# Kyubyong/dc_tts

Hardware: NVIDIA H100
Metric: mel_frames_per_sec (higher is better)
Workload: dtype f32 (decode: fp32 FMA; TextEnc/SSRN: fp16x2 split operands on wgmma, fp32 accumulate)

## Files before the change

### dc_tts_b200/csrc/kernels_decode.cu

```cuda
#include "kernels_decode.cuh"
#include "numerics.cuh"
#include "tc_ptx.cuh"

#include <cuda_fp16.h>
#include <atomic>
#include <cstddef>
#include <math.h>

namespace dctts {
using namespace ptx;

namespace {

constexpr int NC = DEC_NC, GMAX = DEC_GMAX, NT = DEC_THREADS, NWARP = NT / 32;
constexpr int XLD = 768;
constexpr int PLD = GMAX * 32 + 16;
constexpr int TC_RA = DEC_PL_PAD;
constexpr int TC_APLANE = 2 * TC_RA * 16;
constexpr int TC_ASTAGE = 2 * TC_APLANE;
constexpr int TC_NSTG = 6;
constexpr int gcd_c(int a, int b) { return b == 0 ? a : gcd_c(b, a % b); }
constexpr unsigned TC_QCYC = NC / gcd_c(NC, TC_NSTG) * TC_NSTG;
constexpr int TC_PR = 24;
constexpr int TC_PTAP = 2 * 2 * TC_PR * 16;
static_assert(3 * TC_PTAP <= TC_ASTAGE, "packed tap images inside a stage");
static_assert(GMAX * NT >= 1024, "red: LayerNorm parameters of the pre-pass");
static_assert(TC_RA == DEC_PL_PAD, "pl_c1 rows are staged as whole slabs");

struct Smem {
    float ring[DEC_NSLOT][NWARP][DEC_REG_F];
    float red[GMAX][NT];
    float xin[2][GMAX][XLD];
    union {
        float pre[2][NC][PLD];
        unsigned char tca[TC_NSTG][TC_ASTAGE];
    };
    float outv[2][GMAX * 32];
    float prm[2][DEC_PRM_F];
    unsigned long long fullw[DEC_NSLOT][NWARP];
    unsigned long long gbar[2];
    unsigned long long sbar[TC_NSTG], abar[TC_NSTG];
    float stat[GMAX][2][2];
    uint32_t tc_baddr[96];
    int n_moved_frames, n_moved_utt;
    DecParams P;
    int p_cur[GMAX], p_prev[GMAX], p_next[GMAX], moved[GMAX];
    int fmoved[2];
    long long prof[DEC_NPROF], prof_last;
    int stop[GMAX], ulen[GMAX], f_end;
};

static_assert(sizeof(Smem) + 128 <= 232448, "decode kernel: shared memory budget (227 KB per CTA)");
static_assert(offsetof(Smem, tca) + sizeof(Smem::tca) + 128 * 16 <= sizeof(Smem), "A tile reads past the stages");

#define LAP(i) do { if constexpr (PROF) { if (threadIdx.x == 0) { const long long now_ = clock64(); S.prof[i] += now_ - S.prof_last; S.prof_last = now_; } } } while (0)
enum { LP_START = 0, LP_WAIT = 1, LP_GEMV = 2, LP_RELEASE = 3, LP_GATHER = 4, LP_CBAR = 5, LP_LN = 6, LP_MIX = 7, LP_ATT = 8,
       LP_PYR_ATT = 9, LP_PYR_WTS = 10, LP_PYR_TABLE = 11, LP_PYR_STAGE = 12, LP_PYR_DRAIN = 13, LP_PYR_REFILL = 14,
       LP_PYR_LN = 15, LP_PYR_BAR = 16, LP_FRAME = 17,
       LP_WG_AWAIT = 18, LP_WG_MMA = 19, LP_WG_EPI = 20, LP_COUNT };
static_assert(LP_COUNT <= DEC_NPROF, "lap buckets");

__device__ __forceinline__ float sigmoid_fast(float x) { return __fdividef(1.0f, 1.0f + __expf(-x)); }

__device__ __forceinline__ void cp_async16(void* dst, const void* src, bool valid) {
    const int sz = valid ? 16 : 0;
    asm volatile("cp.async.cg.shared.global [%0], [%1], 16, %2;" :: "r"(smem_u32(dst)), "l"(src), "r"(sz) : "memory");
}
__device__ __forceinline__ void cp_async_commit() { asm volatile("cp.async.commit_group;" ::: "memory"); }
template <int N> __device__ __forceinline__ void cp_async_wait() { asm volatile("cp.async.wait_group %0;" :: "n"(N) : "memory"); }

__device__ __forceinline__ void bulk_g2s(void* dst, const void* src, uint32_t bytes, unsigned long long* bar) {
    asm volatile("cp.async.bulk.shared::cluster.global.mbarrier::complete_tx::bytes [%0], [%1], %2, [%3];"
                 :: "r"(smem_u32(dst)), "l"(src), "r"(bytes), "r"(smem_u32(bar)) : "memory");
}
__device__ __forceinline__ void bulk_g2s_mc(void* dst, const void* src, uint32_t bytes, unsigned long long* bar, uint16_t mask) {
    asm volatile("cp.async.bulk.shared::cluster.global.mbarrier::complete_tx::bytes.multicast::cluster [%0], [%1], %2, [%3], %4;"
                 :: "r"(smem_u32(dst)), "l"(src), "r"(bytes), "r"(smem_u32(bar)), "h"(mask) : "memory");
}
__device__ __forceinline__ void bulk_s2peer(uint32_t dst_cluster, const void* src, uint32_t bytes, uint32_t bar_cluster) {
    asm volatile("cp.async.bulk.shared::cluster.shared::cta.mbarrier::complete_tx::bytes [%0], [%1], %2, [%3];"
                 :: "r"(dst_cluster), "r"(smem_u32(src)), "r"(bytes), "r"(bar_cluster) : "memory");
}
__device__ __forceinline__ void cluster_sync_all() { cluster_arrive(); cluster_wait(); }
__device__ __forceinline__ void fence_proxy_async_global() { asm volatile("fence.proxy.async.global;" ::: "memory"); }

__device__ __forceinline__ size_t pl_idx(int nslab, int rows, int b, int c, int t) {
    return ((size_t)(b * nslab + (c >> 4)) * 4 + ((c >> 3) & 1)) * (size_t)rows * 8 + (size_t)(t + DEC_PL_PAD) * 8 + (c & 7);
}
__device__ __forceinline__ float2 ffma2(float2 a, float2 b, float2 c) { return make_float2(fmaf(a.x, b.x, c.x), fmaf(a.y, b.y, c.y)); }
__device__ __forceinline__ float4 ldcg4(const float* p) { return __ldcg(reinterpret_cast<const float4*>(p)); }
__device__ __forceinline__ uint64_t* bar64(unsigned long long* p) { return reinterpret_cast<uint64_t*>(p); }

struct Cur { int f, seg, c; };
__device__ __forceinline__ void cur_next(const DecParams& P, const Smem& S, Cur& u) {
    u.c++;
    const int end = (u.seg == 0) ? P.nch_enc : (u.seg == 1 ? P.pyr_ch1 : P.nch);
    if (u.c < end) return;
    if (u.seg == 0) {
        if (S.fmoved[u.f & 1]) { u.seg = 1; u.c = P.pyr_ch0; } else { u.seg = 2; u.c = P.nch_enc; }
    } else if (u.seg == 1) { u.seg = 2; u.c = P.nch_enc; }
    else { u.f++; u.seg = 0; u.c = 0; }
}
struct Stream {
    const float* base;
    Cur prod;
    unsigned pos;
    unsigned tcq;
};
template <bool STOP>
__device__ __forceinline__ void stream_issue(const DecParams& P, Smem& S, const Stream& st, const Cur& u, int slot, int warp) {
    if (u.f >= (STOP ? S.f_end : P.steps)) return;
    const DecChunk& ch = P.C[u.c];
    const uint32_t bytes = (uint32_t)ch.nfl4 * 2u;
    mbar_expect_tx(bar64(&S.fullw[slot][warp]), bytes);
    const int off = (u.seg == 1) ? ch.off16 : ch.off;
    bulk_g2s(&S.ring[slot][warp][0], st.base + off + warp * (ch.nfl4 >> 1), bytes, &S.fullw[slot][warp]);
}
__device__ __forceinline__ void stream_advance(const DecParams& P, const Smem& S, Stream& st) {
    cur_next(P, S, st.prod); st.pos++;
}
template <bool STOP>
__device__ __forceinline__ void warp_release(const DecParams& P, Smem& S, Stream& st, int warp, int lane) {
    __syncwarp();
    if (lane == 0) stream_issue<STOP>(P, S, st, st.prod, (int)(st.pos % DEC_NSLOT), warp);
    stream_advance(P, S, st);
}

__device__ __forceinline__ void prefetch_params(const DecParams& P, Smem& S, int li, int rank) {
    const DecLayer& l = P.L[li];
    float* dst = S.prm[li & 1];
    const int tid = threadIdx.x;
    cp_async16(dst + tid * 4, P.lnp[li] + tid * 4, true);
    if ((l.cs & 3) == 0) {
        if (tid < l.ns / 4) {
            const int n = tid * 4;
            cp_async16(dst + 1024 + n, P.bias[li] + ((l.kind == 1 && n >= l.cs) ? l.cout + rank * l.cs + (n - l.cs) : rank * l.cs + n), true);
        }
    } else if (tid < l.ns) {
        dst[1024 + tid] = (tid < l.cs) ? __ldg(P.bias[li] + rank * l.cs + tid) : 0.f;
    }
}
__device__ __forceinline__ void prefetch_taps(const DecParams& P, Smem& S, int li, int j, int b0, int G, int buf) {
    const DecLayer& l = P.L[li];
    if (l.ntaps != 3 || !P.in_hist[li]) return;
    for (int i = threadIdx.x; i < G * 128; i += NT) {
        const int c4 = i & 63, tap = (i >> 6) & 1, g = i >> 7;
        const int t = j - (2 - tap) * l.rate;
        const float* src = P.in_hist[li] + ((size_t)(b0 + g) * P.T + (t < 0 ? 0 : t)) * 256 + c4 * 4;
        cp_async16(&S.xin[buf][g][tap * 256 + c4 * 4], src, t >= 0);
    }
}

template <int GT>
__device__ __forceinline__ void gemv_warp(const float* __restrict__ wreg, const float* __restrict__ x, int kr8, int ns, float (&acc)[GT]) {
    const int lane = threadIdx.x & 31;
    const int lg = (ns == 32) ? 5 : (ns == 16 ? 4 : 3);
    const int n = lane & (ns - 1), sg = lane >> lg;
    const int kper = kr8 >> (5 - lg);
    const float* w = wreg + ((size_t)((sg * kper) >> 2) * ns + n) * 4;
    const float* xs = x + sg * kper;
    const int wstep = ns * 4;
    float2 p0[GT], p1[GT];
#pragma unroll
    for (int g = 0; g < GT; ++g) { p0[g] = make_float2(acc[g], 0.f); p1[g] = make_float2(0.f, 0.f); }
#pragma unroll 2
    for (int k = 0; k < kper; k += 8) {
        const float4 w0 = *reinterpret_cast<const float4*>(w);
        const float4 w1 = *reinterpret_cast<const float4*>(w + wstep);
        w += 2 * wstep;
#pragma unroll
        for (int g = 0; g < GT; ++g) {
            const float4 x0 = *reinterpret_cast<const float4*>(xs + g * XLD + k);
            const float4 x1 = *reinterpret_cast<const float4*>(xs + g * XLD + k + 4);
            float2 a = p0[g], c = p1[g];
            a = ffma2(make_float2(x0.x, x0.y), make_float2(w0.x, w0.y), a);
            c = ffma2(make_float2(x1.x, x1.y), make_float2(w1.x, w1.y), c);
            a = ffma2(make_float2(x0.z, x0.w), make_float2(w0.z, w0.w), a);
            c = ffma2(make_float2(x1.z, x1.w), make_float2(w1.z, w1.w), c);
            p0[g] = a; p1[g] = c;
        }
    }
#pragma unroll
    for (int g = 0; g < GT; ++g) acc[g] = (p0[g].x + p0[g].y) + (p1[g].x + p1[g].y);
}


template <int GT>
__device__ __forceinline__ void gemv_warp32(const float* __restrict__ wreg, const float* __restrict__ x, int kr8, float2 (&pe)[GT],
                                            float2 (&po)[GT]) {
    const int lane = threadIdx.x & 31, cp = lane & 15, kh = lane >> 4;
    const float* w = wreg + (kh * 16 + cp) * 4;
    const float* xs = x + kh * 4;
#pragma unroll 2
    for (int k = 0; k < kr8; k += 8) {
        const float4 wa = *reinterpret_cast<const float4*>(w);
        const float4 wb = *reinterpret_cast<const float4*>(w + 128);
        w += 256;
#pragma unroll
        for (int g = 0; g < GT; ++g) {
            const float4 xv = *reinterpret_cast<const float4*>(xs + g * XLD + k);
            float2 a = pe[g], c = po[g];
            a = ffma2(make_float2(xv.x, xv.y), make_float2(wa.x, wa.y), a);
            c = ffma2(make_float2(xv.x, xv.y), make_float2(wb.x, wb.y), c);
            a = ffma2(make_float2(xv.z, xv.w), make_float2(wa.z, wa.w), a);
            c = ffma2(make_float2(xv.z, xv.w), make_float2(wb.z, wb.w), c);
            pe[g] = a; po[g] = c;
        }
    }
}


template <bool PROF, int GT, bool STOP>
__device__ __forceinline__ int layer_row(const DecParams& P, Smem& S, Stream& st, int li, int j, int b0, int G, int rank, int cb, unsigned& lcount) {
    const DecLayer& l = P.L[li];
    const int tid = threadIdx.x, warp = tid >> 5, lane = tid & 31;
    const bool last = (li + 1 == P.nl);
    const int nl_next = last ? 0 : li + 1;
    const int pb = (int)(lcount & 1u);
    const uint32_t gpar = (lcount >> 1) & 1u;
    const uint32_t gbytes = (uint32_t)(GT * l.ns * 4);

    cp_async_wait<0>();
    __syncthreads();
    if (tid == 0) mbar_expect_tx(bar64(&S.gbar[pb]), NC * gbytes);
    if (!last || j + 1 < P.steps) {
        prefetch_params(P, S, nl_next, rank);
        if (nl_next != P.n_enc) prefetch_taps(P, S, nl_next, last ? j + 1 : j, b0, G, cb ^ 1);
    }
    cp_async_commit();
    LAP(LP_START);

    if (l.ns == 32) {
        float2 pe[GT], po[GT];
#pragma unroll
        for (int g = 0; g < GT; ++g) { pe[g] = make_float2(0.f, 0.f); po[g] = make_float2(0.f, 0.f); }
        for (int c = 0; c < l.nch; ++c) {
            const DecChunk& ch = P.C[l.ch0 + c];
            const int slot = (int)(st.pos % DEC_NSLOT);
            mbar_wait(bar64(&S.fullw[slot][warp]), (st.pos / DEC_NSLOT) & 1u);
            LAP(LP_WAIT);
            const int kr8 = ch.krows >> 3;
            gemv_warp32<GT>(&S.ring[slot][warp][0], &S.xin[cb][0][ch.k0 + warp * kr8], kr8, pe, po);
            LAP(LP_GEMV);
            warp_release<STOP>(P, S, st, warp, lane);
            LAP(LP_RELEASE);
        }
#pragma unroll
        for (int g = 0; g < GT; ++g) {
            float e = pe[g].x + pe[g].y, o = po[g].x + po[g].y;
            e += __shfl_xor_sync(0xffffffffu, e, 16);
            o += __shfl_xor_sync(0xffffffffu, o, 16);
            if (lane < 16) *reinterpret_cast<float2*>(&S.red[g][warp * 32 + 2 * lane]) = make_float2(e, o);
        }
    } else {
        float acc[GT];
#pragma unroll
        for (int g = 0; g < GT; ++g) acc[g] = 0.f;
        for (int c = 0; c < l.nch; ++c) {
            const DecChunk& ch = P.C[l.ch0 + c];
            const int slot = (int)(st.pos % DEC_NSLOT);
            mbar_wait(bar64(&S.fullw[slot][warp]), (st.pos / DEC_NSLOT) & 1u);
            LAP(LP_WAIT);
            const int kr8 = ch.krows >> 3;
            gemv_warp<GT>(&S.ring[slot][warp][0], &S.xin[cb][0][ch.k0 + warp * kr8], kr8, l.ns, acc);
            LAP(LP_GEMV);
            warp_release<STOP>(P, S, st, warp, lane);
            LAP(LP_RELEASE);
        }
#pragma unroll
        for (int g = 0; g < GT; ++g) S.red[g][tid] = acc[g];
    }
    __syncthreads();
    const int lgns = (l.ns == 32) ? 5 : (l.ns == 16 ? 4 : 3);
    {
        const int nvals = GT << lgns, ng = NT >> lgns;
        float* ov = S.outv[pb];
        if (tid < nvals) {
            const float* bs = S.prm[li & 1] + 1024;
            const int g = tid >> lgns, n = tid & (l.ns - 1);
            const float* rp = &S.red[g][n];
            float s0 = bs[n], s1 = 0.f;
#pragma unroll 4
            for (int q = 0; q < ng; q += 2) { s0 += rp[q << lgns]; s1 += rp[(q + 1) << lgns]; }
            ov[tid] = s0 + s1;
            fence_proxy_async_smem();
        }
        if (GT > 1) __syncthreads(); else __syncwarp();
        if (tid < NC)
            bulk_s2peer(mapa(smem_u32(&S.pre[pb][rank][0]), (uint32_t)tid), ov, gbytes, mapa(smem_u32(&S.gbar[pb]), (uint32_t)tid));
    }
    LAP(LP_GATHER);
    mbar_wait(bar64(&S.gbar[pb]), gpar);
    LAP(LP_CBAR);
    {
        const int C = l.cout, cs = l.cs, nh = l.kind + 1;
        const float rC = (C == 256) ? (1.0f / 256.0f) : __frcp_rn((float)C);
        auto pre_off = [&](int c) { const int rk = (cs == 16) ? (c >> 4) : ((c * 205) >> 10); return rk * PLD + (c - rk * cs); };
        for (int pr = warp; pr < GT * nh; pr += NWARP) {
            const int g = (nh == 2) ? (pr >> 1) : pr, hf = (nh == 2) ? (pr & 1) : 0;
            const float* base = &S.pre[pb][0][(g << lgns) + hf * cs];
            const float piv = base[0];
            float sv = 0.f, qv = 0.f;
#pragma unroll
            for (int i = 0; i < 8; ++i) {
                const int c = lane + 32 * i;
                if (c < C) { const float d = base[pre_off(c)] - piv; sv += d; qv = fmaf(d, d, qv); }
            }
#pragma unroll
            for (int o = 16; o > 0; o >>= 1) { sv += __shfl_xor_sync(0xffffffffu, sv, o); qv += __shfl_xor_sync(0xffffffffu, qv, o); }
            if (lane == 0) {
                const float m = sv * rC;
                S.stat[g][hf][0] = piv + m;
                S.stat[g][hf][1] = rsqrtf(fmaxf(qv * rC - m * m, 0.f) + 1e-12f);
            }
        }
        __syncthreads();
        LAP(LP_LN);
        const float* prm = S.prm[li & 1];
        const int cur_off = (l.ntaps - 1) * 256;
        const int next_off = (last || li + 1 == P.n_enc) ? 0 : (P.L[li + 1].ntaps - 1) * 256;
        float* oh = P.out_hist[li];
        __half* pl = last ? nullptr : P.pl_hist[li + 1];
        const int c = tid;
        if (c < C) {
            const int po = pre_off(c);
            const bool mine = (po / PLD == rank) && oh;
            const size_t pl_lo = (size_t)P.pl_rows * 16;
            const float g1 = prm[c], b1 = prm[256 + c], g2 = prm[512 + c], b2 = prm[768 + c];
            float o[GT];
#pragma unroll
            for (int g = 0; g < GT; ++g) {
                const float* pr = &S.pre[pb][0][g << lgns];
                o[g] = (pr[po] - S.stat[g][0][0]) * S.stat[g][0][1] * g1 + b1;
            }
            if (l.kind == 1) {
#pragma unroll
                for (int g = 0; g < GT; ++g) {
                    const float* pr = &S.pre[pb][0][g << lgns];
                    const float h2 = (pr[po + cs] - S.stat[g][1][0]) * S.stat[g][1][1] * g2 + b2;
                    const float h1 = sigmoid_fast(o[g]);
                    o[g] = h1 * h2 + (1.0f - h1) * S.xin[cb][g][cur_off + c];
                }
            } else if (l.act == 1) {
#pragma unroll
                for (int g = 0; g < GT; ++g) o[g] = fmaxf(o[g], 0.f);
            }
#pragma unroll
            for (int g = 0; g < GT; ++g) {
                const size_t row = (size_t)(b0 + g) * P.T + j;
                if (mine && g < G) {
                    oh[row * C + c] = o[g];
                    if (pl) {
                        const size_t ix = pl_idx(C >> 4, P.pl_rows, b0 + g, c, j);
                        split_f16(o[g], pl[ix], pl[ix + pl_lo]);
                    }
                }
                if (last) {
                    o[g] = sigmoid_fast(o[g]);
                    if (rank == 0 && g < G) P.ybuf[row * C + c] = o[g];
                }
                S.xin[cb ^ 1][g][next_off + c] = (g < G) ? o[g] : 0.f;
            }
        } else if (last && c < 128) {
#pragma unroll
            for (int g = 0; g < GT; ++g) S.xin[cb ^ 1][g][c] = 0.f;
        }
    }
    LAP(LP_MIX);
    lcount++;
    return cb ^ 1;
}

__device__ __forceinline__ int attend_row(const DecParams& P, const float (&qv)[8], int b, int p, int lane, float (&ctx)[8]) {
    const int d = P.d;
    const int n_lo = min(max(p, 0), P.N - 1), n_hi = min(n_lo + P.win_size, P.N);
    const float scale = rsqrtf((float)d);
    float sc[4] = {0.f, 0.f, 0.f, 0.f};
#pragma unroll
    for (int i = 0; i < 4; ++i) {
        const int n = n_lo + i;
        if (n < n_hi) {
            const float* k = P.kv + ((size_t)b * P.N + n) * (2 * d) + lane * 8;
            const float4 k0 = ldcg4(k), k1 = ldcg4(k + 4);
            float s = 0.f;
            s = fmaf(qv[0], k0.x, s); s = fmaf(qv[1], k0.y, s); s = fmaf(qv[2], k0.z, s); s = fmaf(qv[3], k0.w, s);
            s = fmaf(qv[4], k1.x, s); s = fmaf(qv[5], k1.y, s); s = fmaf(qv[6], k1.z, s); s = fmaf(qv[7], k1.w, s);
            sc[i] = warp_sum(s) * scale;
        }
    }
    const int cnt = n_hi - n_lo;
    float mx = -INFINITY;
#pragma unroll
    for (int i = 0; i < 4; ++i) if (i < cnt) mx = fmaxf(mx, sc[i]);
    float sum = 0.f;
#pragma unroll
    for (int i = 0; i < 4; ++i) if (i < cnt) { sc[i] = expf(sc[i] - mx); sum += sc[i]; }
    float best = -1.f; int besti = 0;
#pragma unroll
    for (int i = 0; i < 4; ++i) if (i < cnt) { sc[i] = sc[i] / sum; if (sc[i] > best) { best = sc[i]; besti = i; } }
#pragma unroll
    for (int i = 0; i < 8; ++i) ctx[i] = 0.f;
#pragma unroll
    for (int i = 0; i < 4; ++i) {
        const int n = n_lo + i;
        if (n < n_hi) {
            const float* v = P.kv + ((size_t)b * P.N + n) * (2 * d) + d + lane * 8;
            const float4 v0 = ldcg4(v), v1 = ldcg4(v + 4);
            const float p_ = sc[i];
            ctx[0] = fmaf(p_, v0.x, ctx[0]); ctx[1] = fmaf(p_, v0.y, ctx[1]); ctx[2] = fmaf(p_, v0.z, ctx[2]); ctx[3] = fmaf(p_, v0.w, ctx[3]);
            ctx[4] = fmaf(p_, v1.x, ctx[4]); ctx[5] = fmaf(p_, v1.y, ctx[5]); ctx[6] = fmaf(p_, v1.z, ctx[6]); ctx[7] = fmaf(p_, v1.w, ctx[7]);
        }
    }
    return n_lo + besti;
}

struct PreRows { unsigned mask; int t_lo, n, total; };
__device__ __forceinline__ PreRows pre_rows(const Smem& S, int G, int j, int prow) {
    PreRows r;
    r.mask = 0;
#pragma unroll
    for (int g = 0; g < GMAX; ++g) if (g < G && S.moved[g]) r.mask |= 1u << g;
    r.t_lo = max(0, j - (prow - 1));
// ... 520 lines not shown
```

### dc_tts_b200/csrc/tc_ptx.cuh

```cuda
#pragma once
#include <cuda_runtime.h>
#include <stdint.h>

namespace dctts { namespace ptx {

__device__ __forceinline__ uint32_t smem_u32(const void* p) {
    return static_cast<uint32_t>(__cvta_generic_to_shared(p));
}
__device__ __forceinline__ bool elect_one() {
    uint32_t pred = 0;
    asm volatile("{\n\t.reg .pred P;\n\telect.sync _|P, 0xffffffff;\n\tselp.u32 %0, 1, 0, P;\n\t}" : "=r"(pred));
    return pred != 0;
}

__device__ __forceinline__ void mbar_init(uint64_t* bar, uint32_t count) {
    asm volatile("mbarrier.init.shared::cta.b64 [%0], %1;" :: "r"(smem_u32(bar)), "r"(count));
}
__device__ __forceinline__ void fence_mbar_init() { asm volatile("fence.mbarrier_init.release.cluster;" ::: "memory"); }
__device__ __forceinline__ void mbar_expect_tx(uint64_t* bar, uint32_t bytes) {
    asm volatile("mbarrier.arrive.expect_tx.shared::cta.b64 _, [%0], %1;" :: "r"(smem_u32(bar)), "r"(bytes) : "memory");
}
__device__ __forceinline__ bool mbar_try_wait(uint64_t* bar, uint32_t parity) {
    uint32_t ok;
    asm volatile(
        "{\n\t.reg .pred P;\n\t"
        "mbarrier.try_wait.parity.shared::cta.b64 P, [%1], %2;\n\t"
        "selp.u32 %0, 1, 0, P;\n\t}"
        : "=r"(ok) : "r"(smem_u32(bar)), "r"(parity) : "memory");
    return ok != 0;
}
__device__ __forceinline__ void mbar_wait(uint64_t* bar, uint32_t parity) {
    if (mbar_try_wait(bar, parity)) return;
    const long long t0 = clock64();
    while (!mbar_try_wait(bar, parity))
        if (clock64() - t0 > 4000000000ll) __trap();
}

__device__ __forceinline__ void prefetch_tmap(const void* tmap) {
    asm volatile("prefetch.tensormap [%0];" :: "l"(reinterpret_cast<uint64_t>(tmap)) : "memory");
}
__device__ __forceinline__ void tma_load_2d(const void* tmap, uint64_t* bar, void* dst, int c0, int c1) {
    asm volatile("cp.async.bulk.tensor.2d.shared::cluster.global.mbarrier::complete_tx::bytes [%0], [%1, {%3, %4}], [%2];"
                 :: "r"(smem_u32(dst)), "l"(reinterpret_cast<uint64_t>(tmap)), "r"(smem_u32(bar)), "r"(c0), "r"(c1)
                 : "memory");
}
__device__ __forceinline__ void tma_load_3d(const void* tmap, uint64_t* bar, void* dst, int c0, int c1, int c2) {
    asm volatile("cp.async.bulk.tensor.3d.shared::cluster.global.mbarrier::complete_tx::bytes [%0], [%1, {%3, %4, %5}], [%2];"
                 :: "r"(smem_u32(dst)), "l"(reinterpret_cast<uint64_t>(tmap)), "r"(smem_u32(bar)), "r"(c0), "r"(c1), "r"(c2)
                 : "memory");
}

__device__ __forceinline__ void tma_load_3d_mc(const void* tmap, uint64_t* bar, void* dst, int c0, int c1, int c2, uint16_t mask) {
    asm volatile("cp.async.bulk.tensor.3d.shared::cluster.global.mbarrier::complete_tx::bytes.multicast::cluster [%0], [%1, {%3, %4, %5}], [%2], %6;"
                 :: "r"(smem_u32(dst)), "l"(reinterpret_cast<uint64_t>(tmap)), "r"(smem_u32(bar)), "r"(c0), "r"(c1), "r"(c2), "h"(mask)
                 : "memory");
}

__device__ __forceinline__ void tma_store_3d(const void* tmap, const void* src, int c0, int c1, int c2) {
    asm volatile("cp.async.bulk.tensor.3d.global.shared::cta.bulk_group [%0, {%2, %3, %4}], [%1];"
                 :: "l"(reinterpret_cast<uint64_t>(tmap)), "r"(smem_u32(src)), "r"(c0), "r"(c1), "r"(c2) : "memory");
}
__device__ __forceinline__ void tma_store_commit_and_wait() {
    asm volatile("cp.async.bulk.commit_group;" ::: "memory");
    asm volatile("cp.async.bulk.wait_group.read 0;" ::: "memory");
}
__device__ __forceinline__ void fence_proxy_async_smem() { asm volatile("fence.proxy.async.shared::cta;" ::: "memory"); }

__device__ __forceinline__ void wg_fence() { asm volatile("wgmma.fence.sync.aligned;" ::: "memory"); }
__device__ __forceinline__ void wg_commit() { asm volatile("wgmma.commit_group.sync.aligned;" ::: "memory"); }
template <int N>
__device__ __forceinline__ void wg_wait() { asm volatile("wgmma.wait_group.sync.aligned %0;" :: "n"(N) : "memory"); }
template <int R>
__device__ __forceinline__ void wg_fence_regs(float (&d)[R]) {
#pragma unroll
    for (int i = 0; i < R; ++i) asm volatile("" : "+f"(d[i]) :: "memory");
}

#define DCTTS_WG_D8(o) "+f"(d[o + 0]), "+f"(d[o + 1]), "+f"(d[o + 2]), "+f"(d[o + 3]), "+f"(d[o + 4]), "+f"(d[o + 5]), "+f"(d[o + 6]), "+f"(d[o + 7])
template <int NQ, int R>
__device__ __forceinline__ void wgmma_f16(float (&d)[R], uint64_t da, uint64_t db, uint32_t accumulate) {
    static_assert(NQ >= 1 && NQ <= 4 && 8 * NQ <= R, "wgmma_f16: 16..64 columns");
    if constexpr (NQ == 1) {
        asm volatile("{\n\t.reg .pred p;\n\tsetp.ne.b32 p, %10, 0;\n\t"
                     "wgmma.mma_async.sync.aligned.m64n16k16.f32.f16.f16 {%0,%1,%2,%3,%4,%5,%6,%7}, %8, %9, p, 1, 1, 0, 0;\n\t}"
                     : DCTTS_WG_D8(0) : "l"(da), "l"(db), "r"(accumulate));
    } else if constexpr (NQ == 2) {
        asm volatile("{\n\t.reg .pred p;\n\tsetp.ne.b32 p, %18, 0;\n\t"
                     "wgmma.mma_async.sync.aligned.m64n32k16.f32.f16.f16 {%0,%1,%2,%3,%4,%5,%6,%7,%8,%9,%10,%11,%12,%13,%14,%15},"
                     " %16, %17, p, 1, 1, 0, 0;\n\t}"
                     : DCTTS_WG_D8(0), DCTTS_WG_D8(8) : "l"(da), "l"(db), "r"(accumulate));
    } else if constexpr (NQ == 3) {
        asm volatile("{\n\t.reg .pred p;\n\tsetp.ne.b32 p, %26, 0;\n\t"
                     "wgmma.mma_async.sync.aligned.m64n48k16.f32.f16.f16 {%0,%1,%2,%3,%4,%5,%6,%7,%8,%9,%10,%11,%12,%13,%14,%15,"
                     "%16,%17,%18,%19,%20,%21,%22,%23}, %24, %25, p, 1, 1, 0, 0;\n\t}"
                     : DCTTS_WG_D8(0), DCTTS_WG_D8(8), DCTTS_WG_D8(16) : "l"(da), "l"(db), "r"(accumulate));
    } else {
        asm volatile("{\n\t.reg .pred p;\n\tsetp.ne.b32 p, %34, 0;\n\t"
                     "wgmma.mma_async.sync.aligned.m64n64k16.f32.f16.f16 {%0,%1,%2,%3,%4,%5,%6,%7,%8,%9,%10,%11,%12,%13,%14,%15,"
                     "%16,%17,%18,%19,%20,%21,%22,%23,%24,%25,%26,%27,%28,%29,%30,%31}, %32, %33, p, 1, 1, 0, 0;\n\t}"
                     : DCTTS_WG_D8(0), DCTTS_WG_D8(8), DCTTS_WG_D8(16), DCTTS_WG_D8(24) : "l"(da), "l"(db), "r"(accumulate));
    }
}
template <int N>
__device__ __forceinline__ void wgmma_full(float (&d)[N / 2], uint64_t da, uint64_t db, uint32_t accumulate) {
    static_assert(N == 64 || N == 80 || N == 144 || N == 256, "wgmma_full: unsupported width");
    if constexpr (N == 64) {
        asm volatile("{\n\t.reg .pred p;\n\tsetp.ne.b32 p, %34, 0;\n\t"
                     "wgmma.mma_async.sync.aligned.m64n64k16.f32.f16.f16 {%0,%1,%2,%3,%4,%5,%6,%7,%8,%9,%10,%11,%12,%13,%14,%15,%16,%17,%18,%19,%20,%21,%22,%23,%24,%25,%26,%27,%28,%29,%30,%31},"
                     " %32, %33, p, 1, 1, 0, 0;\n\t}"
                     : DCTTS_WG_D8(0), DCTTS_WG_D8(8), DCTTS_WG_D8(16), DCTTS_WG_D8(24) : "l"(da), "l"(db), "r"(accumulate));
    } else if constexpr (N == 80) {
        asm volatile("{\n\t.reg .pred p;\n\tsetp.ne.b32 p, %42, 0;\n\t"
                     "wgmma.mma_async.sync.aligned.m64n80k16.f32.f16.f16 {%0,%1,%2,%3,%4,%5,%6,%7,%8,%9,%10,%11,%12,%13,%14,%15,%16,%17,%18,%19,%20,%21,%22,%23,%24,%25,%26,%27,%28,%29,%30,%31,%32,%33,%34,%35,%36,%37,%38,%39},"
                     " %40, %41, p, 1, 1, 0, 0;\n\t}"
                     : DCTTS_WG_D8(0), DCTTS_WG_D8(8), DCTTS_WG_D8(16), DCTTS_WG_D8(24), DCTTS_WG_D8(32) : "l"(da), "l"(db), "r"(accumulate));
    } else if constexpr (N == 144) {
        asm volatile("{\n\t.reg .pred p;\n\tsetp.ne.b32 p, %74, 0;\n\t"
                     "wgmma.mma_async.sync.aligned.m64n144k16.f32.f16.f16 {%0,%1,%2,%3,%4,%5,%6,%7,%8,%9,%10,%11,%12,%13,%14,%15,%16,%17,%18,%19,%20,%21,%22,%23,%24,%25,%26,%27,%28,%29,%30,%31,%32,%33,%34,%35,%36,%37,%38,%39,%40,%41,%42,%43,%44,%45,%46,%47,%48,%49,%50,%51,%52,%53,%54,%55,%56,%57,%58,%59,%60,%61,%62,%63,%64,%65,%66,%67,%68,%69,%70,%71},"
// ... 76 lines not shown
```

### dc_tts_b200/engine.py

```python
import ctypes as C
import warnings

import numpy as np
import torch

from . import _lib
from .hyperparams import Hyperparams as hp
from .params import check_params


class DcttsError(RuntimeError):
    pass


def _ptr(t):
    return C.c_void_p(0) if t is None else C.c_void_p(t.data_ptr())


def _require_tensors(who, want):
    for t, shape, dt in want:
        if tuple(t.shape) != shape or t.dtype != dt or not t.is_cuda or not t.is_contiguous():
            raise DcttsError("%s: expected a contiguous CUDA %s tensor of shape %s, got %s %s" %
                             (who, dt, shape, t.dtype, tuple(t.shape)))

# ... 11 lines not shown
        h = _lib.Handle()
        torch.cuda.init()
        with torch.cuda.device(self.device):
            torch.zeros(1, device=self.device)
            rc = self._lib.dctts_create(C.byref(st), device, C.byref(h))
        if rc != 0:
            raise DcttsError("dctts_create: " + self._lib.dctts_last_error(None).decode())
        self._h = h
        self.params_loaded = False

    def close(self):
        if getattr(self, "_h", None):
            self._lib.dctts_destroy(self._h)
            self._h = None

    def __del__(self):
        try:
            self.close()
        except Exception:
            pass

    def _check(self, rc, what):
        if rc != 0:
            raise DcttsError("%s: %s" % (what, self._lib.dctts_last_error(self._h).decode()))

    def _stream(self):
        return C.c_void_p(torch.cuda.current_stream(self.device).cuda_stream)

    def _f32(self, x):
        if isinstance(x, np.ndarray):
            x = torch.from_numpy(np.ascontiguousarray(x, dtype=np.float32))
        return x.to(device=self.device, dtype=torch.float32).contiguous()

    def _i32(self, x):
        if isinstance(x, np.ndarray):
            x = torch.from_numpy(np.ascontiguousarray(x, dtype=np.int32))
        return torch.as_tensor(x).to(device=self.device, dtype=torch.int32).contiguous()

    def _empty(self, *shape, dtype=torch.float32):
        return torch.empty(shape, device=self.device, dtype=dtype)

    def stage_params(self, params):
        for name, arr in params.items():
            a = np.ascontiguousarray(arr, dtype=np.float32)
            shape = (C.c_int64 * a.ndim)(*a.shape)
            self._check(self._lib.dctts_set_param(self._h, name.encode(), a.ctypes.data_as(C.c_void_p),
                                                   shape, a.ndim), "dctts_set_param(%s)" % name)

    def commit_params(self):
        self._check(self._lib.dctts_commit_params(self._h), "dctts_commit_params")
        self.params_loaded = True
        return int(self._lib.dctts_num_params(self._h))

    def load_params(self, params):
        check_params(params)
        self.stage_params(params)
        return self.commit_params()

    def restore(self, text2mel_dir, ssrn_dir=None):
        from .checkpoint import Saver, latest_checkpoint
        Saver(var_list=["Text2Mel"]).restore(self, latest_checkpoint(text2mel_dir))
        Saver(var_list=["SSRN", "gs"]).restore(self, latest_checkpoint(ssrn_dir if ssrn_dir is not None else text2mel_dir))
        return self.commit_params()

    def set_tensor_path(self, mode):
        self._check(self._lib.dctts_set_tensor_path(self._h, int(mode)), "dctts_set_tensor_path")

    def set_option(self, name, value):
        self._check(self._lib.dctts_set_option(self._h, name.encode(), int(value)), "dctts_set_option(%s)" % name)

    def get_option(self, name):
        v = C.c_int32(0)
        self._check(self._lib.dctts_get_option(self._h, name.encode(), C.byref(v)), "dctts_get_option(%s)" % name)
        return int(v.value)

    def decode_stats(self):
        a, b, c = C.c_int32(0), C.c_int32(0), C.c_int32(0)
        self._check(self._lib.dctts_decode_stats(self._h, C.byref(a), C.byref(b), C.byref(c)), "dctts_decode_stats")
        return int(a.value), int(b.value), int(c.value)

    def decode_profile(self):
        names = ["start", "stream_wait", "gemv", "release", "gather", "cluster_barrier", "layernorm", "mix", "attention",
                 "re_attention", "re_weights", "re_table", "re_stage", "re_drain", "re_refill", "re_layernorm", "re_barriers",
                 "frame", "wg_a_wait", "wg_mma", "wg_epilogue"]
        v = (C.c_int64 * len(names))()
        self._check(self._lib.dctts_decode_profile(self._h, v, len(names)), "dctts_decode_profile")
        return dict(zip(names, [int(x) for x in v]))

    def reserve(self, batch):
        self._check(self._lib.dctts_reserve(self._h, int(batch)), "dctts_reserve")

    def bench_block(self, scope, B, L, iters=5, warmup=2):
        ms = (C.c_float * 8)()
        n = C.c_int32(0)
        self._check(self._lib.dctts_bench_block(self._h, scope.encode(), B, L, iters, warmup, ms, C.byref(n),
                                                self._stream()), "dctts_bench_block")
        return [float(ms[i]) for i in range(n.value)]

    def conv_gemm(self, impl, mode, X, K, Wd, N, shifts, out, bias=None, accumulate=0):
        ts = [X, Wd, out] + ([bias] if bias is not None else [])
        if not all(t.is_cuda and t.dtype == torch.float32 and t.stride(-1) == 1 for t in ts):
            raise DcttsError("conv_gemm: CUDA float32 tensors with a unit inner stride expected")
        B, L = X.shape[0], X.shape[1]
        rows_ok = X.stride(0) == L * X.stride(1) and (mode == 1 or out.stride(0) == L * out.stride(1))
        taps_ok = (Wd.stride(0) == K * Wd.stride(1)) if mode == 0 else (out.stride(0) == K * out.stride(1))
        dy_ok = mode == 0 or (Wd.shape[0] == B and Wd.shape[1] == L and Wd.stride(0) == L * Wd.stride(1))
        if not (rows_ok and taps_ok and dy_ok):
            raise DcttsError("conv_gemm: rows or taps of a tensor are not evenly pitched")
        sh = (C.c_int32 * len(shifts))(*[int(s) for s in shifts])
        self._check(self._lib.dctts_conv_gemm(self._h, int(impl), int(mode), _ptr(X), X.stride(1), B, L, int(K), _ptr(Wd),
                                              Wd.stride(1), int(N), len(shifts), sh, _ptr(bias), int(accumulate), _ptr(out),
                                              out.stride(1), self._stream()), "dctts_conv_gemm")
        return out

    @staticmethod
    def _pitched(who, ts, rows):
        if not all(t.is_cuda and t.dtype == torch.float32 and t.stride(-1) == 1 for t in ts):
            raise DcttsError("%s: CUDA float32 tensors with a unit inner stride expected" % who)
        pitches = []
        for t in ts:
            lead = t.shape[:-1]
            n = 1
            for s in lead:
                n *= s
            ld = t.stride(-2) if t.dim() >= 2 else t.shape[-1]
            even = all(t.stride(i) == t.stride(i + 1) * t.shape[i + 1] for i in range(t.dim() - 2))
            if n != rows or not even:
                raise DcttsError("%s: rows of a tensor are not evenly pitched, or not %d of them" % (who, rows))
            pitches.append(ld)
        return pitches

    def block_bwd(self, mode, act, C, pre, gout, ln, dy, dparams, X=None, gin=None, dropout_rate=0.0, layer=0, seed=0):
        nconv = 2 * C if mode == 1 else C
        if mode == 1 and (X is None or gin is None):
            raise DcttsError("block_bwd: a highway block (mode 1) needs X and gin")
        rows = 1
        for s in pre.shape[:-1]:
            rows *= s
        ts = [pre, gout, dy] + ([X, gin] if mode == 1 else [])
        if any(t.shape[-1] < w for t, w in zip(ts, (nconv, C, nconv, C, C))):
            raise DcttsError("block_bwd: pre and dy need %d columns, gout, X and gin %d" % (nconv, C))
        lds = self._pitched("block_bwd", ts, rows)
        if gout.stride(-2) != lds[1] or (mode == 1 and gin.stride(-2) != lds[1]):
            raise DcttsError("block_bwd: gout and gin share one pitch")
        if dy.stride(-2) != lds[0]:
            raise DcttsError("block_bwd: pre and dy share one pitch")
        _require_tensors("block_bwd", [(ln, (4, C), torch.float32), (dparams, (4 * C + nconv,), torch.float32)])
        self._check(self._lib.dctts_block_bwd(self._h, int(mode), int(act), rows, int(C), _ptr(pre), lds[0], _ptr(gout), lds[1],
                                              _ptr(X), lds[3] if mode == 1 else 0, _ptr(ln), float(dropout_rate), int(layer),
                                              int(seed) & 0xffffffff, _ptr(dy), _ptr(gin), _ptr(dparams), self._stream()),
                    "dctts_block_bwd")
        return dy

    def attn_bwd(self, gR, Q, KV, align, gts, n_lim, t_lim, gQ, gKV, sums):
        B, T, N, d = align.shape[0], align.shape[2], align.shape[1], self.hp.d
        f32 = torch.float32
        _require_tensors("attn_bwd", [(gR, (B, T, 2 * d), f32), (Q, (B, T, d), f32), (KV, (B, N, 2 * d), f32),
                                      (align, (B, N, T), f32), (gQ, (B, T, d), f32), (gKV, (B, N, 2 * d), f32),
                                      (sums, (3,), torch.float64)])
        if gts.dim() != 2 or gts.shape[0] < n_lim or gts.shape[1] < t_lim:
            raise DcttsError("attn_bwd: gts must be 2-D with at least n_lim = %d rows and t_lim = %d columns, got %s"
                             % (n_lim, t_lim, tuple(gts.shape)))
        ld_gts = self._pitched("attn_bwd", [gts], gts.shape[0])[0]
        self._check(self._lib.dctts_attn_bwd(self._h, _ptr(gR), _ptr(Q), _ptr(KV), _ptr(align), _ptr(gts), ld_gts, B, T, N,
                                             int(n_lim), int(t_lim), _ptr(gQ), _ptr(gKV), _ptr(sums), self._stream()),
                    "dctts_attn_bwd")
        return gQ, gKV
# ... 492 lines not shown
```

Before: 141,100.

## Scatter decode partials with st.async and merge LayerNorm stats per rank

Replaces the staged outv buffer and bulk shared-to-peer copy with direct per-thread st.async pushes of the reduced values into every cluster rank's pre buffer. Each rank also computes local mean/M2 partials via warp shuffles and sends them, so the LayerNorm statistics are merged with a Chan-style combine instead of a separate warp pass, a __syncthreads and a stat array. Parameter and tap prefetch is moved after the gather so it overlaps the cluster barrier wait, which now uses a cluster-scope acquire. This trades a block barrier and an smem round-trip for many small remote stores and extra shuffle work.

```diff
diff --git a/dc_tts_b200/csrc/kernels_decode.cu b/dc_tts_b200/csrc/kernels_decode.cu
--- a/dc_tts_b200/csrc/kernels_decode.cu
+++ b/dc_tts_b200/csrc/kernels_decode.cu
@@ -15,6 +15,7 @@
 constexpr int NC = DEC_NC, GMAX = DEC_GMAX, NT = DEC_THREADS, NWARP = NT / 32;
 constexpr int XLD = 768;
 constexpr int PLD = GMAX * 32 + 16;
+constexpr int PPD = 2 * NC + 4;
 constexpr int TC_RA = DEC_PL_PAD;
 constexpr int TC_APLANE = 2 * TC_RA * 16;
 constexpr int TC_ASTAGE = 2 * TC_APLANE;
@@ -32,15 +33,16 @@
     float red[GMAX][NT];
     float xin[2][GMAX][XLD];
     union {
-        float pre[2][NC][PLD];
+        struct {
+            float pre[2][NC][PLD];
+            float part[2][GMAX * 2][PPD];
+        };
         unsigned char tca[TC_NSTG][TC_ASTAGE];
     };
-    float outv[2][GMAX * 32];
     float prm[2][DEC_PRM_F];
     unsigned long long fullw[DEC_NSLOT][NWARP];
     unsigned long long gbar[2];
     unsigned long long sbar[TC_NSTG], abar[TC_NSTG];
-    float stat[GMAX][2][2];
     uint32_t tc_baddr[96];
     int n_moved_frames, n_moved_utt;
     DecParams P;
@@ -52,12 +54,15 @@
 
 static_assert(sizeof(Smem) + 128 <= 232448, "decode kernel: shared memory budget (227 KB per CTA)");
 static_assert(offsetof(Smem, tca) + sizeof(Smem::tca) + 128 * 16 <= sizeof(Smem), "A tile reads past the stages");
+static_assert(offsetof(Smem, pre) % 16 == 0 && (PLD * 4) % 16 == 0, "pre: 16-byte st.async targets");
+static_assert(offsetof(Smem, part) % 16 == 0 && (PPD * 4) % 16 == 0, "part: float4 loads of the merge");
 
 #define LAP(i) do { if constexpr (PROF) { if (threadIdx.x == 0) { const long long now_ = clock64(); S.prof[i] += now_ - S.prof_last; S.prof_last = now_; } } } while (0)
 enum { LP_START = 0, LP_WAIT = 1, LP_GEMV = 2, LP_RELEASE = 3, LP_GATHER = 4, LP_CBAR = 5, LP_LN = 6, LP_MIX = 7, LP_ATT = 8,
        LP_PYR_ATT = 9, LP_PYR_WTS = 10, LP_PYR_TABLE = 11, LP_PYR_STAGE = 12, LP_PYR_DRAIN = 13, LP_PYR_REFILL = 14,
        LP_PYR_LN = 15, LP_PYR_BAR = 16, LP_FRAME = 17,
-       LP_WG_AWAIT = 18, LP_WG_MMA = 19, LP_WG_EPI = 20, LP_COUNT };
+       LP_WG_AWAIT = 18, LP_WG_MMA = 19, LP_WG_EPI = 20,
+       LP_PREFETCH = 21, LP_COUNT };
 static_assert(LP_COUNT <= DEC_NPROF, "lap buckets");
 
 __device__ __forceinline__ float sigmoid_fast(float x) { return __fdividef(1.0f, 1.0f + __expf(-x)); }
@@ -76,10 +81,6 @@
 __device__ __forceinline__ void bulk_g2s_mc(void* dst, const void* src, uint32_t bytes, unsigned long long* bar, uint16_t mask) {
     asm volatile("cp.async.bulk.shared::cluster.global.mbarrier::complete_tx::bytes.multicast::cluster [%0], [%1], %2, [%3], %4;"
                  :: "r"(smem_u32(dst)), "l"(src), "r"(bytes), "r"(smem_u32(bar)), "h"(mask) : "memory");
-}
-__device__ __forceinline__ void bulk_s2peer(uint32_t dst_cluster, const void* src, uint32_t bytes, uint32_t bar_cluster) {
-    asm volatile("cp.async.bulk.shared::cluster.shared::cta.mbarrier::complete_tx::bytes [%0], [%1], %2, [%3];"
-                 :: "r"(dst_cluster), "r"(smem_u32(src)), "r"(bytes), "r"(bar_cluster) : "memory");
 }
 __device__ __forceinline__ void cluster_sync_all() { cluster_arrive(); cluster_wait(); }
 __device__ __forceinline__ void fence_proxy_async_global() { asm volatile("fence.proxy.async.global;" ::: "memory"); }
@@ -218,16 +219,12 @@
     const int nl_next = last ? 0 : li + 1;
     const int pb = (int)(lcount & 1u);
     const uint32_t gpar = (lcount >> 1) & 1u;
-    const uint32_t gbytes = (uint32_t)(GT * l.ns * 4);
+    const int nh = l.kind + 1;
+    const uint32_t gbytes = (uint32_t)(GT * l.ns * 4), pbytes = (uint32_t)(GT * nh * 8);
 
     cp_async_wait<0>();
     __syncthreads();
-    if (tid == 0) mbar_expect_tx(bar64(&S.gbar[pb]), NC * gbytes);
-    if (!last || j + 1 < P.steps) {
-        prefetch_params(P, S, nl_next, rank);
-        if (nl_next != P.n_enc) prefetch_taps(P, S, nl_next, last ? j + 1 : j, b0, G, cb ^ 1);
-    }
-    cp_async_commit();
+    if (tid == 0) mbar_expect_tx(bar64(&S.gbar[pb]), NC * (gbytes + pbytes));
     LAP(LP_START);
 
     if (l.ns == 32) {
@@ -272,50 +269,88 @@
     }
     __syncthreads();
     const int lgns = (l.ns == 32) ? 5 : (l.ns == 16 ? 4 : 3);
+    const int cs = l.cs;
     {
         const int nvals = GT << lgns, ng = NT >> lgns;
-        float* ov = S.outv[pb];
-        if (tid < nvals) {
-            const float* bs = S.prm[li & 1] + 1024;
+        if ((tid & ~31) < nvals) {
             const int g = tid >> lgns, n = tid & (l.ns - 1);
-            const float* rp = &S.red[g][n];
-            float s0 = bs[n], s1 = 0.f;
+            float v = 0.f;
+            if (tid < nvals) {
+                const float* bs = S.prm[li & 1] + 1024;
+                const float* rp = &S.red[g][n];
+                float s0 = bs[n], s1 = 0.f;
 #pragma unroll 4
-            for (int q = 0; q < ng; q += 2) { s0 += rp[q << lgns]; s1 += rp[(q + 1) << lgns]; }
-            ov[tid] = s0 + s1;
-            fence_proxy_async_smem();
-        }
-        if (GT > 1) __syncthreads(); else __syncwarp();
-        if (tid < NC)
-            bulk_s2peer(mapa(smem_u32(&S.pre[pb][rank][0]), (uint32_t)tid), ov, gbytes, mapa(smem_u32(&S.gbar[pb]), (uint32_t)tid));
+                for (int q = 0; q < ng; q += 2) { s0 += rp[q << lgns]; s1 += rp[(q + 1) << lgns]; }
+                v = s0 + s1;
+            }
+            const int W = (l.ns == 8) ? 8 : 16, w = lane & (W - 1);
+            const float piv = __shfl_sync(0xffffffffu, v, lane & ~(W - 1));
+            const float d = (w < cs) ? v - piv : 0.f;
+            float s1 = d, s2 = d * d;
+#pragma unroll
+            for (int o = 1; o < 8; o <<= 1) { s1 += __shfl_xor_sync(0xffffffffu, s1, o); s2 += __shfl_xor_sync(0xffffffffu, s2, o); }
+            if (W == 16) { s1 += __shfl_xor_sync(0xffffffffu, s1, 8); s2 += __shfl_xor_sync(0xffffffffu, s2, 8); }
+            const float md = s1 * ((cs == 16) ? (1.0f / 16.0f) : __frcp_rn((float)cs));
+            const float mr = piv + md, m2 = fmaxf(fmaf(-s1, md, s2), 0.f);
+            const int q0 = lane & ~3;
+            const float4 v4 = make_float4(__shfl_sync(0xffffffffu, v, q0), __shfl_sync(0xffffffffu, v, q0 + 1),
+                                          __shfl_sync(0xffffffffu, v, q0 + 2), __shfl_sync(0xffffffffu, v, q0 + 3));
+            if (tid < nvals) {
+                const uint32_t bar = smem_u32(&S.gbar[pb]);
+                const uint32_t vdst = smem_u32(&S.pre[pb][rank][(g << lgns) + (n & ~3)]);
+                const int hf = (l.ns == 32) ? (n >> 4) : 0;
+                const uint32_t pdst = smem_u32(&S.part[pb][2 * g + hf][2 * rank]);
+#pragma unroll
+                for (int i = 0; i < NC / 4; ++i) {
+                    const uint32_t r = (uint32_t)((lane & 3) + 4 * i);
+                    st_async_v4(mapa(vdst, r), v4, mapa(bar, r));
+                }
+                for (int r = w; r < NC; r += W) st_async_v2(mapa(pdst, (uint32_t)r), mr, m2, mapa(bar, (uint32_t)r));
+            }
+        }
     }
     LAP(LP_GATHER);
-    mbar_wait(bar64(&S.gbar[pb]), gpar);
+    if (!last || j + 1 < P.steps) {
+        prefetch_params(P, S, nl_next, rank);
+        if (nl_next != P.n_enc) prefetch_taps(P, S, nl_next, last ? j + 1 : j, b0, G, cb ^ 1);
+    }
+    cp_async_commit();
+    LAP(LP_PREFETCH);
+    mbar_wait_cluster(bar64(&S.gbar[pb]), gpar);
     LAP(LP_CBAR);
     {
-        const int C = l.cout, cs = l.cs, nh = l.kind + 1;
+        const int C = l.cout;
         const float rC = (C == 256) ? (1.0f / 256.0f) : __frcp_rn((float)C);
+        float mu = 0.f, rs = 0.f;
+        if (lane < 2 * GT && (lane & 1) < nh) {
+            const float* pp = &S.part[pb][lane][0];
+            float4 a[NC / 2];
+#pragma unroll
+            for (int i = 0; i < NC / 2; ++i) a[i] = *reinterpret_cast<const float4*>(pp + 4 * i);
+            const float m0 = a[0].x;
+            float sd0 = 0.f, sd1 = 0.f;
+#pragma unroll
+            for (int i = 0; i < NC / 2; ++i) { sd0 += a[i].x - m0; sd1 += a[i].z - m0; }
+            mu = m0 + (sd0 + sd1) * (1.0f / NC);
+            float q0 = 0.f, q1 = 0.f, e0 = 0.f, e1 = 0.f;
+#pragma unroll
+            for (int i = 0; i < NC / 2; ++i) {
+                const float d0 = a[i].x - mu, d1 = a[i].z - mu;
+                q0 += a[i].y; q1 += a[i].w;
+                e0 = fmaf(d0, d0, e0); e1 = fmaf(d1, d1, e1);
+            }
+            rs = rsqrtf(fmaxf(fmaf((float)cs, e0 + e1, q0 + q1) * rC, 0.f) + 1e-12f);
+        }
+        float mean[GT][2], rstd[GT][2];
+#pragma unroll
+        for (int g = 0; g < GT; ++g)
+#pragma unroll
+            for (int hf = 0; hf < 2; ++hf) {
+                mean[g][hf] = __shfl_sync(0xffffffffu, mu, 2 * g + hf);
+                rstd[g][hf] = __shfl_sync(0xffffffffu, rs, 2 * g + hf);
+            }
+        LAP(LP_LN);
         auto pre_off = [&](int c) { const int rk = (cs == 16) ? (c >> 4) : ((c * 205) >> 10); return rk * PLD + (c - rk * cs); };
-        for (int pr = warp; pr < GT * nh; pr += NWARP) {
-            const int g = (nh == 2) ? (pr >> 1) : pr, hf = (nh == 2) ? (pr & 1) : 0;
-            const float* base = &S.pre[pb][0][(g << lgns) + hf * cs];
-            const float piv = base[0];
-            float sv = 0.f, qv = 0.f;
-#pragma unroll
-            for (int i = 0; i < 8; ++i) {
-                const int c = lane + 32 * i;
-                if (c < C) { const float d = base[pre_off(c)] - piv; sv += d; qv = fmaf(d, d, qv); }
-            }
-#pragma unroll
-            for (int o = 16; o > 0; o >>= 1) { sv += __shfl_xor_sync(0xffffffffu, sv, o); qv += __shfl_xor_sync(0xffffffffu, qv, o); }
-            if (lane == 0) {
-                const float m = sv * rC;
-                S.stat[g][hf][0] = piv + m;
-                S.stat[g][hf][1] = rsqrtf(fmaxf(qv * rC - m * m, 0.f) + 1e-12f);
-            }
-        }
-        __syncthreads();
-        LAP(LP_LN);
         const float* prm = S.prm[li & 1];
         const int cur_off = (l.ntaps - 1) * 256;
         const int next_off = (last || li + 1 == P.n_enc) ? 0 : (P.L[li + 1].ntaps - 1) * 256;
@@ -331,13 +366,13 @@
 #pragma unroll
             for (int g = 0; g < GT; ++g) {
                 const float* pr = &S.pre[pb][0][g << lgns];
-                o[g] = (pr[po] - S.stat[g][0][0]) * S.stat[g][0][1] * g1 + b1;
+                o[g] = (pr[po] - mean[g][0]) * rstd[g][0] * g1 + b1;
             }
             if (l.kind == 1) {
 #pragma unroll
                 for (int g = 0; g < GT; ++g) {
                     const float* pr = &S.pre[pb][0][g << lgns];
-                    const float h2 = (pr[po + cs] - S.stat[g][1][0]) * S.stat[g][1][1] * g2 + b2;
+                    const float h2 = (pr[po + cs] - mean[g][1]) * rstd[g][1] * g2 + b2;
                     const float h1 = sigmoid_fast(o[g]);
                     o[g] = h1 * h2 + (1.0f - h1) * S.xin[cb][g][cur_off + c];
                 }
diff --git a/dc_tts_b200/csrc/tc_ptx.cuh b/dc_tts_b200/csrc/tc_ptx.cuh
--- a/dc_tts_b200/csrc/tc_ptx.cuh
+++ b/dc_tts_b200/csrc/tc_ptx.cuh
@@ -34,6 +34,29 @@
     const long long t0 = clock64();
     while (!mbar_try_wait(bar, parity))
         if (clock64() - t0 > 4000000000ll) __trap();
+}
+__device__ __forceinline__ bool mbar_try_wait_cluster(uint64_t* bar, uint32_t parity) {
+    uint32_t ok;
+    asm volatile(
+        "{\n\t.reg .pred P;\n\t"
+        "mbarrier.try_wait.parity.acquire.cluster.shared::cta.b64 P, [%1], %2;\n\t"
+        "selp.u32 %0, 1, 0, P;\n\t}"
+        : "=r"(ok) : "r"(smem_u32(bar)), "r"(parity) : "memory");
+    return ok != 0;
+}
+__device__ __forceinline__ void mbar_wait_cluster(uint64_t* bar, uint32_t parity) {
+    if (mbar_try_wait_cluster(bar, parity)) return;
+    const long long t0 = clock64();
+    while (!mbar_try_wait_cluster(bar, parity))
+        if (clock64() - t0 > 4000000000ll) __trap();
+}
+__device__ __forceinline__ void st_async_v4(uint32_t dst, float4 v, uint32_t bar) {
+    asm volatile("st.async.shared::cluster.mbarrier::complete_tx::bytes.v4.f32 [%0], {%1, %2, %3, %4}, [%5];"
+                 :: "r"(dst), "f"(v.x), "f"(v.y), "f"(v.z), "f"(v.w), "r"(bar) : "memory");
+}
+__device__ __forceinline__ void st_async_v2(uint32_t dst, float a, float b, uint32_t bar) {
+    asm volatile("st.async.shared::cluster.mbarrier::complete_tx::bytes.v2.f32 [%0], {%1, %2}, [%3];"
+                 :: "r"(dst), "f"(a), "f"(b), "r"(bar) : "memory");
 }
 
 __device__ __forceinline__ void prefetch_tmap(const void* tmap) {
diff --git a/dc_tts_b200/engine.py b/dc_tts_b200/engine.py
--- a/dc_tts_b200/engine.py
+++ b/dc_tts_b200/engine.py
@@ -117,7 +117,7 @@
     def decode_profile(self):
         names = ["start", "stream_wait", "gemv", "release", "gather", "cluster_barrier", "layernorm", "mix", "attention",
                  "re_attention", "re_weights", "re_table", "re_stage", "re_drain", "re_refill", "re_layernorm", "re_barriers",
-                 "frame", "wg_a_wait", "wg_mma", "wg_epilogue"]
+                 "frame", "wg_a_wait", "wg_mma", "wg_epilogue", "prefetch"]
         v = (C.c_int64 * len(names))()
         self._check(self._lib.dctts_decode_profile(self._h, v, len(names)), "dctts_decode_profile")
         return dict(zip(names, [int(x) for x in v]))
```

After: 147,700 (median of 6 runs). 1.05x the previous value.
